# blacksnail789521/IMM-TSF

Measured on AMD Instinct MI355X. Metric: forecast windows/sec (train fwd+bwd) on ragged 64-entity batch, higher is better.
Workload: dtype bf16

## Files before the change

imm-tsf_amd/csrc/capi.hip:

```cpp
#include "../../include/immtsf.h"
#include "attn.hpp"
#include "gemm.hpp"
#include "rowops.hpp"
#include "tail.hpp"
#include "block_util.hpp"
#include <atomic>

namespace {
inline DropCfg mk_drop(float p, uint64_t seed) {
    DropCfg d;
    d.seed = seed;
    d.p = p > 0.f ? p : 0.f;
    d.inv_keep = d.p > 0.f ? 1.f / (1.f - d.p) : 1.f;
    d.seed_dev = nullptr;
    return d;
}
}

namespace { std::atomic<int> g_side_enabled{0}; }

extern "C" {

int immtsf_side_stream_enabled(void) { return g_side_enabled; }
int immtsf_set_side_stream(int32_t on) { g_side_enabled.store(on ? 1 : 0); return 0; }

int immtsf_gemm(int32_t layout, int32_t precision, const float* A, int32_t lda, const float* B, int32_t ldb, float* C,
                int32_t ldc, const float* bias, int32_t M, int32_t N, int32_t K, float alpha, int32_t accumulate,
                int32_t act, immtsf_stream_t stream) {
    if (!A || !B || !C || layout < 0 || layout > 2) return IMMTSF_EINVAL;
    GemmArgs g = gemm_args(M, N, K, lda, ldb, ldc);
    set_problem(g, 0, A, B, C, bias);
    g.alpha = alpha;
    g.accumulate = accumulate;
    g.act = act;
    return immtsf_launch_gemm(layout, precision, g, static_cast<hipStream_t>(stream));
}

int immtsf_linear_backward(int32_t precision, const float* x, const float* W, const float* dy, int32_t M, int32_t N,
                           int32_t K, float* dx, const float* relu_x, float* dW, float* db, int32_t grads_prezeroed,
                           immtsf_stream_t stream) {
    if (!dy || M <= 0 || N <= 0 || K <= 0 || (db && !dW) || (dx && !W) || (dW && !x)) return IMMTSF_EINVAL;
    hipStream_t s = static_cast<hipStream_t>(stream);
    if (linear_small_ok(M, N, K) && (!dW || grads_prezeroed)) return launch_linear_small_bwd(x, W, dy, M, N, K, dx, relu_x, dW, db, s);
    if (dx) {
        GemmArgs g = gemm_args(M, K, N, N, K, K);
        set_problem(g, 0, dy, W, dx, nullptr);
        g.relu_ref = relu_x;
        g.ld_ref = K;
        if (int rc = immtsf_launch_gemm(GEMM_NN, precision, g, s)) return rc;
    }
    if (dW) {
        GemmArgs g = gemm_args(N, K, M, N, K, K);
        set_problem(g, 0, dy, x, dW, nullptr, db);
        g.c_prezeroed = grads_prezeroed ? 1 : 0;
        if (int rc = immtsf_launch_gemm(GEMM_TN, precision, g, s)) return rc;
    }
// ... 78 lines not shown
    return launch_bf16_to_f32(src, dst, n, static_cast<hipStream_t>(stream));
}

int immtsf_gemm_batched(int32_t layout, int32_t precision, const float* A, int32_t lda, int64_t sA_o, int64_t sA_i,
                        const float* B, int32_t ldb, int64_t sB_o, int64_t sB_i, float* C, int32_t ldc, int64_t sC_o,
                        int64_t sC_i, int32_t n_outer, int32_t n_inner, int32_t M, int32_t N, int32_t K, float alpha,
                        immtsf_stream_t stream) {
    if (!A || !B || !C || layout < 0 || layout > 2 || n_outer <= 0 || n_inner <= 0) return IMMTSF_EINVAL;
    GemmArgs g = gemm_args(M, N, K, lda, ldb, ldc);
    set_problem(g, 0, A, B, C, nullptr);
    g.alpha = alpha;
    g.nbatch = n_outer * n_inner;
    g.batch_inner = n_inner;
    g.sA_o = sA_o; g.sA_i = sA_i; g.sB_o = sB_o; g.sB_i = sB_i; g.sC_o = sC_o; g.sC_i = sC_i;
    if (g.nbatch == 1) { g.nbatch = 1; }
    return immtsf_launch_gemm(layout, precision, g, static_cast<hipStream_t>(stream));
}

int immtsf_softmax_rows_forward(float* sc, float* A, int32_t B, int32_t H, int32_t L, int32_t S, const uint8_t* live,
                                float p_drop, uint64_t seed, uint64_t site, int32_t causal, const uint64_t* seed_step_dev,
                                immtsf_stream_t stream) {
    if (!sc || !A) return IMMTSF_EINVAL;
    DropCfg d = mk_drop(p_drop, seed);
    d.seed_dev = seed_step_dev;
    return launch_softmax_rows_fwd(sc, A, B, H, L, S, live, d, site, causal, static_cast<hipStream_t>(stream));
}

int immtsf_softmax_rows_backward(float* dA, const float* P, int32_t B, int32_t H, int32_t L, int32_t S, float p_drop,
                                 uint64_t seed, uint64_t site, const uint64_t* seed_step_dev, immtsf_stream_t stream) {
    if (!dA || !P) return IMMTSF_EINVAL;
    DropCfg d = mk_drop(p_drop, seed);
    d.seed_dev = seed_step_dev;
    return launch_softmax_rows_bwd(dA, P, B, H, L, S, d, site, static_cast<hipStream_t>(stream));
}

int immtsf_attention_short_forward(const float* qkv, int32_t B, int32_t L, int32_t H, int32_t E, float scale, int32_t causal,
                                   float p_drop, uint64_t seed, uint64_t site, const uint64_t* seed_step_dev, float* out,
                                   immtsf_stream_t stream) {
    if (!qkv || !out || B < 0 || L <= 0 || H <= 0 || E <= 0) return IMMTSF_EINVAL;
    DropCfg d = mk_drop(p_drop, seed);
    d.seed_dev = seed_step_dev;
    return launch_attn_short_fwd(qkv, B, L, H, E, scale, causal, d, site, out, static_cast<hipStream_t>(stream));
}

int immtsf_attention_short_backward(const float* qkv, const float* dout, int32_t B, int32_t L, int32_t H, int32_t E, float scale,
                                    int32_t causal, float p_drop, uint64_t seed, uint64_t site, const uint64_t* seed_step_dev,
                                    float* dqkv, immtsf_stream_t stream) {
    if (!qkv || !dout || !dqkv || B < 0 || L <= 0 || H <= 0 || E <= 0) return IMMTSF_EINVAL;
    DropCfg d = mk_drop(p_drop, seed);
    d.seed_dev = seed_step_dev;
    return launch_attn_short_bwd(qkv, dout, B, L, H, E, scale, causal, d, site, dqkv, static_cast<hipStream_t>(stream));
}

int immtsf_layernorm_forward(const float* x, int32_t rows, int32_t d, const float* gamma, const float* beta, float eps,
                             float* xhat, float* rstd, float* z, float p_drop, uint64_t seed, uint64_t site,
                             immtsf_stream_t stream) {
    if (!x || !gamma || !beta || !z || d <= 0) return IMMTSF_EINVAL;
    return launch_layernorm_fwd(x, rows, d, gamma, beta, eps, xhat, rstd, z, mk_drop(p_drop, seed), site,
                                static_cast<hipStream_t>(stream));
}

int immtsf_layernorm_backward(float* dz_dy, int32_t rows, int32_t d, const float* gamma, const float* xhat,
                              const float* rstd, float* dx, float* dgamma, float* dbeta, float* scratch, float p_drop,
                              uint64_t seed, uint64_t site, immtsf_stream_t stream) {
    if (!dz_dy || !gamma || !xhat || !rstd || !dx || d <= 0) return IMMTSF_EINVAL;
    hipStream_t s = static_cast<hipStream_t>(stream);
    CHECK(launch_layernorm_bwd(dz_dy, rows, d, gamma, xhat, rstd, dx, mk_drop(p_drop, seed), site, s));
    if (dgamma && dbeta) {
        if (!scratch) return IMMTSF_EINVAL;
        return launch_colsum2(dz_dy, xhat, rows, d, d, dgamma, dbeta, scratch, s);
    }
    if (dgamma) {
        if (!scratch) return IMMTSF_EINVAL;
        CHECK(launch_colsum(dz_dy, xhat, rows, nullptr, d, d, dgamma, 0, scratch, s));
    }
    if (dbeta) {
        if (!scratch) return IMMTSF_EINVAL;
        CHECK(launch_colsum(dz_dy, nullptr, rows, nullptr, d, d, dbeta, 0, scratch, s));
    }
    return IMMTSF_OK;
}

int immtsf_dropout_mask(uint64_t seed, uint64_t site, uint64_t n, float p_drop, uint8_t* out, immtsf_stream_t stream) {
    if (!out) return IMMTSF_EINVAL;
    return launch_dropout_mask(seed, site, (size_t)n, p_drop, out, static_cast<hipStream_t>(stream));
}

int immtsf_masked_mse_sums(const float* truth, const float* pred, const float* mask, int32_t rows, int32_t C,
                           float* err_sum, float* cnt, float* scratch, immtsf_stream_t stream) {
    if (!truth || !pred || !mask || !err_sum || !cnt || !scratch || rows < 0 || C <= 0) return IMMTSF_EINVAL;
    return launch_mse_sums(truth, pred, mask, rows, C, err_sum, cnt, scratch, static_cast<hipStream_t>(stream));
}

int immtsf_masked_mse(const float* truth, const float* pred, const float* mask, int32_t rows, int32_t C, const float* cnt_global,
                      float* err_sum, float* cnt, float* loss, float* dpred, float grad_scale, immtsf_stream_t stream) {
    if (!truth || !pred || !mask || !loss || rows < 0 || C <= 0) return IMMTSF_EINVAL;
    if ((int64_t)rows * C > IMMTSF_MSE_SMALL_MAX || C > 4096) return IMMTSF_EUNSUPPORTED;
    return launch_mse_small(truth, pred, mask, rows, C, cnt_global, err_sum, cnt, loss, dpred, grad_scale,
                            static_cast<hipStream_t>(stream));
}

int immtsf_masked_mse_counted(const float* truth, const float* pred, const float* mask, int32_t rows, int32_t C, const float* cnt_global,
                              float* scratch, float* loss, float* dpred, float grad_scale, immtsf_stream_t stream) {
    if (!truth || !pred || !mask || !cnt_global || !scratch || !loss || rows < 0 || C <= 0) return IMMTSF_EINVAL;
    if (C > 64) return IMMTSF_EUNSUPPORTED;
    return launch_mse_counted(truth, pred, mask, rows, C, cnt_global, scratch + 1, reinterpret_cast<unsigned int*>(scratch), loss, dpred,
// ... 117 lines not shown
```

imm-tsf_amd/csrc/rowops.hip:

```cpp
#include "rowops.hpp"

namespace {

constexpr int kSlabs = 32;

__global__ __launch_bounds__(256) void note_mask_kernel(const float* __restrict__ V, int rows, int d_m,
                                                         unsigned char* __restrict__ mask, int* nan_flag, int vec) {
    const int lane = threadIdx.x & 63, row = blockIdx.x * 4 + (threadIdx.x >> 6);
    if (row >= rows) return;
    const float* p = V + (size_t)row * d_m;
    float s = 0.f;
    bool bad = false;
    if (vec) {
        const float4* p4 = reinterpret_cast<const float4*>(p);
        for (int i = lane; i < d_m / 4; i += 64) {
            const float4 v = p4[i];
            s += fabsf(v.x) + fabsf(v.y) + fabsf(v.z) + fabsf(v.w);
            bad |= (v.x != v.x) | (v.y != v.y) | (v.z != v.z) | (v.w != v.w);
        }
    } else {
        for (int i = lane; i < d_m; i += 64) {
            const float v = p[i];
            s += fabsf(v);
            bad |= (v != v);
// ... 1484 lines not shown
        hipLaunchKernelGGL(layernorm_bwd_kernel, dim3(cdiv(rows, 4)), dim3(256), 0, s, dz_dy, rows, d, gamma, xhat, rstd, dx, drop,
                           site);
    IMMTSF_LAUNCH_CHECK();
    return IMMTSF_OK;
}

bool ln_sums_compact_ok(int rows, int d) {
    return (d & 3) == 0 && d <= 256 * LN_DV && rows >= 512 && (size_t)3 * 3 * d * sizeof(float) <= 64 * 1024;
}
int launch_layernorm_bwd_sums(float* dz_dy, int rows, int d, const float* gamma, const float* xhat, const float* rstd, float* dx,
                              DropCfg drop, uint64_t site, float* out_gw, float* out_gb, float* out_q, float* scratch,
                              const unsigned char* row_flag, int flag_div, void* dxh, hipStream_t s, const void* xhat_h) {
    if (rows <= 0) return IMMTSF_OK;
    constexpr bool on = true;
    const uintptr_t al = reinterpret_cast<uintptr_t>(dz_dy) | reinterpret_cast<uintptr_t>(dx) | reinterpret_cast<uintptr_t>(xhat) |
                         reinterpret_cast<uintptr_t>(gamma) | reinterpret_cast<uintptr_t>(scratch);
    if (!on || (d & 3) || d > 256 * LN_DV || (al & 15) || ((reinterpret_cast<uintptr_t>(dxh) | reinterpret_cast<uintptr_t>(xhat_h)) & 7) ||
        rows < 512)
        return IMMTSF_EUNSUPPORTED;
    if ((!xhat && !xhat_h) || (!dx && !dxh)) return IMMTSF_EINVAL;
    int nsl = (rows + 3) / 4;
    nsl = nsl > kLnSlabsMax ? kLnSlabsMax : nsl;
    const size_t lds = (size_t)3 * (out_q ? 3 : 2) * d * sizeof(float);
    if (out_q) {
        if (lds > 64 * 1024) return IMMTSF_EUNSUPPORTED;
        if (xhat_h)
            hipLaunchKernelGGL((layernorm_bwd_sums_kernel<3, true>), dim3(nsl), dim3(256), lds, s, dz_dy, rows, d, gamma, xhat_h, rstd, dx, drop, site,
                               scratch, row_flag, flag_div > 0 ? flag_div : 1, static_cast<bf16_t*>(dxh));
        else
            hipLaunchKernelGGL((layernorm_bwd_sums_kernel<3, false>), dim3(nsl), dim3(256), lds, s, dz_dy, rows, d, gamma, xhat, rstd, dx, drop, site,
                               scratch, row_flag, flag_div > 0 ? flag_div : 1, static_cast<bf16_t*>(dxh));
        IMMTSF_LAUNCH_CHECK();
        hipLaunchKernelGGL((colsum_vec_final_kernel<3>), dim3(cdiv(d, 32), 3), dim3(256), 0, s, scratch, d, nsl, out_gw, out_gb, out_q, 0);
    } else {
        if (lds > 64 * 1024 || row_flag || dxh || xhat_h || !dx) return IMMTSF_EUNSUPPORTED;
        hipLaunchKernelGGL((layernorm_bwd_sums_kernel<2, false>), dim3(nsl), dim3(256), lds, s, dz_dy, rows, d, gamma, xhat, rstd, dx, drop, site, scratch,
                           nullptr, 1, nullptr);
        IMMTSF_LAUNCH_CHECK();
        hipLaunchKernelGGL((colsum_vec_final_kernel<2>), dim3(cdiv(d, 32), 2), dim3(256), 0, s, scratch, d, nsl, out_gw, out_gb, nullptr, 0);
    }
    IMMTSF_LAUNCH_CHECK();
    return IMMTSF_OK;
}

int launch_instance_norm(const float* x, int B, int L, int C, float* xn, float* means, float* stdev, hipStream_t s) {
    if (B <= 0 || L <= 0 || C <= 0) return IMMTSF_OK;
    const size_t lds = ((size_t)L * C + 2 * (size_t)C) * sizeof(float);
    if (lds > 64 * 1024) return IMMTSF_EUNSUPPORTED;
    hipLaunchKernelGGL(instance_norm_kernel, dim3(B), dim3(256), lds, s, x, B, L, C, xn, means, stdev);
    IMMTSF_LAUNCH_CHECK();
    return IMMTSF_OK;
}

bool ln_lr_ok(int rows, int d, int PW) {
    return (d & 3) == 0 && d <= 1024 && d >= 256 && PW >= 1 && PW <= 64 && rows >= 512 && (size_t)(PW + 3) * d * sizeof(float) <= 150 * 1024;
}
int launch_layernorm_bwd_lr(const float* G, int ldg, int PW, const float* Wb, int rows, int d, const float* gamma, const float* xhat,
                            const void* xhat_h, const float* rstd, float* dx, void* dxh, DropCfg drop, uint64_t site, float* out_gw, float* out_gb,
                            float* out_q, float* scratch, const unsigned char* row_flag, int flag_div, hipStream_t s, const void* keep, int keep_T) {
    if (!ln_lr_ok(rows, d, PW)) return IMMTSF_EUNSUPPORTED;
    if (keep && (keep_T <= 0 || keep_T > 32)) return IMMTSF_EINVAL;
    if (!G || !Wb || (!xhat && !xhat_h) || (!dx && !dxh) || !out_gw || !out_gb || !out_q || !scratch) return IMMTSF_EINVAL;
    const uintptr_t al = reinterpret_cast<uintptr_t>(Wb) | reinterpret_cast<uintptr_t>(dx) | reinterpret_cast<uintptr_t>(gamma) |
                         reinterpret_cast<uintptr_t>(scratch) | reinterpret_cast<uintptr_t>(xhat);
    if ((al & 15) || ((reinterpret_cast<uintptr_t>(dxh) | reinterpret_cast<uintptr_t>(xhat_h)) & 7)) return IMMTSF_EUNSUPPORTED;
    const void* xa = xhat_h ? xhat_h : static_cast<const void*>(xhat);
    const size_t lds = (size_t)(PW + 3) * d * sizeof(float);
    const bool many = rows >= 8192;
    const int per_wg = 8 * (many ? (d <= 768 ? 4 : 2) : 1);
    int nsl = cdiv(rows, per_wg);
    nsl = nsl > 256 ? 256 : nsl;
    const int fd = flag_div > 0 ? flag_div : 1;
#define LNLR(RR, DVV, XHH)                                                                                                                       \
    do {                                                                                                                                         \
        static const hipError_t attr = hipFuncSetAttribute(reinterpret_cast<const void*>(layernorm_bwd_lr_kernel<RR, DVV, XHH>),                 \
                                                           hipFuncAttributeMaxDynamicSharedMemorySize, 150 * 1024);                              \
        if (attr != hipSuccess) return (int)attr;                                                                                                \
        hipLaunchKernelGGL((layernorm_bwd_lr_kernel<RR, DVV, XHH>), dim3(nsl), dim3(512), lds, s, G, ldg, PW, Wb, rows, d, gamma, xa, rstd, dx,   \
                           static_cast<bf16_t*>(dxh), drop, site, scratch, row_flag, fd, static_cast<const unsigned long long*>(keep), keep_T); \
    } while (0)
#define LNLR2(RR, DVV) do { if (xhat_h) LNLR(RR, DVV, true); else LNLR(RR, DVV, false); } while (0)
    if (d <= 768) { if (many) LNLR2(4, 3); else LNLR2(1, 3); }
    else { if (many) LNLR2(2, 4); else LNLR2(1, 4); }
#undef LNLR2
#undef LNLR
    IMMTSF_LAUNCH_CHECK();
    hipLaunchKernelGGL((colsum_vec_final_kernel<3>), dim3(cdiv(d, 32), 3), dim3(256), 0, s, scratch, d, nsl, out_gw, out_gb, out_q, 0);
    IMMTSF_LAUNCH_CHECK();
    return IMMTSF_OK;
}

int launch_matvec(const float* W, int ldw, const float* x, const float* b, int rows, int cols, float* y, float* ys,
                  float scale, hipStream_t s, float* y_nobias) {
    hipLaunchKernelGGL(matvec_kernel, dim3(cdiv(rows, 4)), dim3(256), 0, s, W, ldw, x, b, rows, cols, y, ys, scale, y_nobias);
    IMMTSF_LAUNCH_CHECK();
    return IMMTSF_OK;
}

int launch_matvec_t(const float* W, int ldw, const float* x, int rows, int cols, float* y, int accumulate,
                    hipStream_t s) {
    const int slabs = (accumulate && rows >= 256) ? 16 : 1;
    hipLaunchKernelGGL(matvec_t_kernel, dim3(cdiv(cols, 64), slabs), dim3(1024), 0, s, W, ldw, x, rows, cols, y, accumulate);
    IMMTSF_LAUNCH_CHECK();
    return IMMTSF_OK;
}

int launch_outer(const float* a, const float* b, int rows, int cols, float* out, int ld, hipStream_t s) {
    const long n = (long)rows * cols;
    hipLaunchKernelGGL(outer_kernel, dim3((unsigned)((n + 255) / 256)), dim3(256), 0, s, a, b, rows, cols, out, ld);
    IMMTSF_LAUNCH_CHECK();
    return IMMTSF_OK;
}

int launch_query_bwd(const float* dqs_part, int B, int d, float scale, const float* Wq, int ldw, const float* Q, float* dWq, int ldg,
                     float* dbq, float* dQ, hipStream_t s) {
    if (d <= 0) return IMMTSF_OK;
    hipLaunchKernelGGL(query_bwd_kernel, dim3(cdiv(d, QB_ROWS)), dim3(256), 0, s, dqs_part, B, d, scale, Wq, ldw, Q,
                       dWq, ldg, dbq, dQ);
    IMMTSF_LAUNCH_CHECK();
    return IMMTSF_OK;
}

int launch_query_t2v_bwd(const float* dqs_part, int B, int d, float scale, const float* Wq, int ldw, const float* Q, float* dWq, int ldg,
                         float* dbq, float* dQ, const float* tau_pad, const int* rowmap, const int* total, int max_rows, int d_tau,
                         const float* w, const float* b, const float* dfeat, int ld, float* dw0, float* db0, float* dw, float* db,
                         float* scratch, int nslabs, hipStream_t s, int accumulate) {
    if (d <= 0 || max_rows <= 0) return IMMTSF_EINVAL;
    if (nslabs < 1) nslabs = kSlabs;
    const int nq = cdiv(d, QB_ROWS), gx = cdiv(d_tau, 64);
    const QueryBwdJob q{dqs_part, B, d, scale, Wq, ldw, Q, dWq, ldg, dbq, dQ};
    const T2VBwdJob t{tau_pad, rowmap, total, d_tau, w, b, dfeat, ld, scratch, max_rows, gx, nslabs};
    hipLaunchKernelGGL(query_t2v_bwd_kernel, dim3(nq + gx * nslabs), dim3(256), 0, s, q, nq, t);
    IMMTSF_LAUNCH_CHECK();
    hipLaunchKernelGGL(time2vec_bwd_final_kernel, dim3(cdiv(d_tau, 4)), dim3(256), 0, s, scratch, d_tau, dw0, db0, dw, db, nslabs, accumulate);
    IMMTSF_LAUNCH_CHECK();
    return IMMTSF_OK;
// ... 90 lines not shown
```

imm-tsf_amd/csrc/rowops.hpp:

```cpp
#pragma once
#include "common.hpp"

int launch_note_mask(const float* V, int rows, int d_m, unsigned char* mask, int* nan_flag, hipStream_t s);
int launch_ragged_index(const unsigned char* mask, int B, int N, int* lengths, int* offsets, int* rowmap, int* seg,
                        unsigned char* mtxt, hipStream_t s, unsigned char* mtxt2 = nullptr);
int launch_mask_from_lengths(const int* lengths, int B, int N, unsigned char* mask, hipStream_t s);
int launch_gather_rows(const float* src, int ld_src, const int* rowmap, const int* total, int max_rows, int width,
                       float* dst, int ld_dst, hipStream_t s, void* dst_h = nullptr);
int launch_time2vec_fwd(const float* tau_pad, const int* rowmap, const int* total, int max_rows, int d_tau,
                        const float* w0, const float* b0, const float* w, const float* b, float* dst, int ld_dst,
                        hipStream_t s, void* dst_h = nullptr);
int launch_notes_stage(const float* src, int ld_src, const int* gmap, const int* total, int max_rows, int width, void* dst_h, int ld_dst,
                       const float* tau_pad, const int* rowmap, int d_tau, const float* w0, const float* b0, const float* w, const float* b,
                       float* t_dst, int t_ld, void* t_dst_h, const float* W, int ldw, const float* x, const float* bias, int rows, int cols,
                       float* y, float* ys, float scale, hipStream_t s,
                       const float* W2 = nullptr, int ldw2 = 0, const float* x2 = nullptr, const float* bias2 = nullptr, int rows2 = 0,
                       int cols2 = 0, float* y2 = nullptr,
                       const float* score_u = nullptr, float* score_out = nullptr);
int launch_query_t2v_bwd(const float* dqs_part, int B, int d, float scale, const float* Wq, int ldw, const float* Q, float* dWq, int ldg,
                         float* dbq, float* dQ, const float* tau_pad, const int* rowmap, const int* total, int max_rows, int d_tau,
                         const float* w, const float* b, const float* dfeat, int ld, float* dw0, float* db0, float* dw, float* db,
                         float* scratch, int nslabs, hipStream_t s, int accumulate = 0);
int launch_time2vec_bwd(const float* tau_pad, const int* rowmap, const int* total, int max_rows, int d_tau,
                        const float* w, const float* b, const float* dfeat, int ld, float* dw0, float* db0, float* dw,
                        float* db, float* scratch, int nslabs, hipStream_t s, int accumulate = 0);
int launch_colsum(const float* X, const float* Y, int M, const int* dyn, int N, int ld, float* out, int accumulate,
                  float* scratch, hipStream_t s, bool big_scratch = false);
bool colsum_small_pair_ok(int M, int N);
int launch_colsum_small_pair(const float* X, const float* Y, const float* Z, int M, int N, int ld, float* out_xy, float* out_x, float* out_z,
                             hipStream_t s, int outputs_zero = 0);
int launch_colsum2(const float* X, const float* Y, int M, int N, int ld, float* out_xy, float* out_x, float* scratch,
                   hipStream_t s, bool big_scratch = false);
inline size_t colsum_scratch_floats(size_t ncols, int k) { return (size_t)256 * k * ((ncols + 3) & ~(size_t)3) + 64 * 8; }
int launch_colsum3(const float* X, const float* Y, float* Z, int M, int N, int ld, float* out_xy, float* out_x, float* out_z,
                   float* scratch, const unsigned char* row_flag, int flag_div, void* Zh, hipStream_t s, bool big_scratch = false);
int launch_layernorm_fwd(const float* x, int rows, int d, const float* gamma, const float* beta, float eps, float* xhat,
                         float* rstd, float* z, DropCfg drop, uint64_t site, hipStream_t s, void* zh = nullptr,
                         const float* res = nullptr, DropCfg pre = DropCfg{0, 0.f, 1.f, nullptr}, uint64_t presite = 0,
                         void* xhat_h = nullptr);
int launch_layernorm_bwd(float* dz_dy, int rows, int d, const float* gamma, const float* xhat, const float* rstd,
                         float* dx, DropCfg drop, uint64_t site, hipStream_t s, float* dbranch = nullptr,
                         DropCfg pre = DropCfg{0, 0.f, 1.f, nullptr}, uint64_t presite = 0);
constexpr int kLnSlabsMax = 2048;
inline size_t ln_sums_scratch_floats(size_t d, int k) { return (size_t)kLnSlabsMax * k * ((d + 3) & ~(size_t)3) + 64 * 8; }
int launch_layernorm_bwd_sums(float* dz_dy, int rows, int d, const float* gamma, const float* xhat, const float* rstd, float* dx,
                              DropCfg drop, uint64_t site, float* out_gw, float* out_gb, float* out_q, float* scratch,
                              const unsigned char* row_flag, int flag_div, void* dxh, hipStream_t s, const void* xhat_h = nullptr);
int launch_instance_norm(const float* x, int B, int L, int C, float* xn, float* means, float* stdev, hipStream_t s);
bool ln_lr_ok(int rows, int d, int PW);
int launch_layernorm_bwd_lr(const float* G, int ldg, int PW, const float* Wb, int rows, int d, const float* gamma, const float* xhat,
                            const void* xhat_h, const float* rstd, float* dx, void* dxh, DropCfg drop, uint64_t site, float* out_gw, float* out_gb,
                            float* out_q, float* scratch, const unsigned char* row_flag, int flag_div, hipStream_t s, const void* keep = nullptr,
                            int keep_T = 0);
bool ln_sums_compact_ok(int rows, int d);
int launch_matvec(const float* W, int ldw, const float* x, const float* b, int rows, int cols, float* y, float* ys,
                  float scale, hipStream_t s, float* y_nobias = nullptr);
int launch_matvec_t(const float* W, int ldw, const float* x, int rows, int cols, float* y, int accumulate,
                    hipStream_t s);
int launch_outer(const float* a, const float* b, int rows, int cols, float* out, int ld, hipStream_t s);
int launch_axpy(const float* src, float alpha, float* dst, int n, int accumulate, hipStream_t s);
int launch_query_bwd(const float* dqs_part, int B, int d, float scale, const float* Wq, int ldw, const float* Q, float* dWq, int ldg,
                     float* dbq, float* dQ, hipStream_t s);
int launch_fill(float* dst, float v, size_t n, hipStream_t s);
int launch_dropout_mask(uint64_t seed, uint64_t site, size_t n, float p, unsigned char* out, hipStream_t s);
bool head_sums_supported(int M, int C);
int launch_head_sums(const float* dn, const float* xhat, const float* ddelta, const unsigned char* flag, int flag_div, int M, int C,
                     float* out_xy, float* out_x, float* slive, hipStream_t s);
int launch_head_outer(const float* Wres, int d, const float* slive, const float* bout, int C, float* dbout, float* dWres, hipStream_t s);
```

imm-tsf_amd/csrc/xrank.hip:

```cpp
#include "../../include/immtsf.h"
#include "gemm.hpp"
#include "rowops.hpp"
#include "tail.hpp"
#include "block_util.hpp"
#include "t2v_fold.hpp"
#include "eval.hpp"
#include <math.h>
#include <algorithm>
#include <vector>
#include <type_traits>

namespace {

constexpr int XR = 8;
constexpr int XJ_MAX = 20;
enum { XJ_NN = 0, XJ_NT = 1, XJ_OUTER = 2, XJ_COPY = 3 };
struct XJob {
    int form, nblk;
    const float* L; int lsr, lsn;
    int R;
    const float* W; int ldw, qsn;
    int K, N, M;
    float* out; int osr, osn;
    unsigned short* out16;
    float alpha;
    const float *lb, *wb;
    const float* radd;
    const float* xrow;
    int ng; long pgs, qgs;
};
struct XJobs { int first[XJ_MAX]; int n; int lds_floats; XJob j[XJ_MAX]; };

__device__ __forceinline__ unsigned short f2bf(float v) {
    return __builtin_bit_cast(unsigned short, static_cast<__bf16>(v));
}

constexpr int XJ_LK = 16 * 1024;

__device__ __forceinline__ bool xjob_stage_l(const XJob& J, float* Ls, int cap) {
    if (J.R * J.K > cap) return false;
    if (J.lsn == 1) {
        for (int i = threadIdx.x; i < J.R * J.K; i += 256) {
            const int r = i / J.K, k = i - r * J.K;
            Ls[i] = J.L[(size_t)r * J.lsr + k];
        }
    } else {
        for (int i = threadIdx.x; i < J.R * J.K; i += 256) {
            const int k = i / J.R, r = i - k * J.R;
            Ls[r * J.K + k] = J.L[(size_t)r * J.lsr + (size_t)k * J.lsn];
        }
    }
    __syncthreads();
    return true;
}

template <bool STAGED>
__device__ __forceinline__ void xjob_nn_acc(const XJob& J, int kg, int n, const float* Ls, float4 (&acc)[XR]) {
    constexpr int U = STAGED ? 8 : 6;
    const int R = J.R;
// ... 1411 lines not shown
    }
    {
        GemmArgs g = gemm_args(BT, x.PW, d, d, d, x.PW);
        set_problem2(g, 0, Em, mat(w.Wf, w.Wf16), mat(P), w.Wfb);
        CHECK(immtsf_launch_gemm(GEMM_NT, prec, g, s));
    }
    return IMMTSF_OK;
}

static int xrank_compose_z(const immtsf_fusion_cfg* cfg, const float* proj_w, const float* proj_b, const XPWs& w, hipStream_t s) {
    const XRDims x = xr_dims(cfg);
    const int d = x.d, prec = cfg->precision;
    const bool hf = xr_hf(cfg);
    Mat Wpo;
    CHECK(weight_mat(hf, proj_w, (size_t)d * d, w.Wpo16, s, &Wpo));
    {
        GemmArgs g = gemm_args(x.PW, d, d, d, d, d);
        set_problem2(g, 0, mat(w.Wf, w.Wf16), Wpo, mat(w.Wc, w.Wc16), nullptr);
        CHECK(immtsf_launch_gemm(GEMM_NN, prec, g, s));
    }
    {
        VecJobList l;
        l.add(VJ_MV, w.Wf, d, proj_b, w.Wfb, w.bc, x.PW, d);
        CHECK(launch_vecjobs(l, s));
    }
    return IMMTSF_OK;
}

int immtsf_mmf_xrank_fold_z(const immtsf_fusion_cfg* cfg, const immtsf_xadd_params* p, const float* proj_w, const float* proj_b, float* bHO,
                            void* workspace, size_t workspace_bytes, immtsf_stream_t stream) {
    if (!proj_w || !proj_b) return IMMTSF_EINVAL;
    CHECK(immtsf_mmf_xrank_fold(cfg, p, bHO, workspace, workspace_bytes, stream));
    return xrank_compose_z(cfg, proj_w, proj_b, carve_xp(cfg, workspace), static_cast<hipStream_t>(stream));
}

int immtsf_mmf_xrank_p_forward_z(const immtsf_fusion_cfg* cfg, const immtsf_xadd_params* p, const float* proj_w, const float* proj_b,
                                 const float* Z, float* P, float* bHO, void* workspace, size_t workspace_bytes, int32_t folded,
                                 immtsf_stream_t stream) {
    if (!xr_supported(cfg) || !p || !proj_w || !proj_b || !Z || !P || !bHO || !workspace) return IMMTSF_EINVAL;
    XPWs w = carve_xp(cfg, workspace);
    if (workspace_bytes < w.bytes) return IMMTSF_EWORKSPACE;
    if (!folded) CHECK(immtsf_mmf_xrank_fold_z(cfg, p, proj_w, proj_b, bHO, workspace, workspace_bytes, stream));
    hipStream_t s = static_cast<hipStream_t>(stream);
    const XRDims x = xr_dims(cfg);
    const int d = x.d, BT = x.B * x.T, prec = cfg->precision;
    const bool hf = xr_hf(cfg);
    Mat Zm = cmat(Z);
    if (hf && cfg->in_h) {
        Zm.h = const_cast<void*>(cfg->in_h);
    } else if (hf) {
        CHECK(launch_f32_to_bf16(Z, w.E16, (size_t)BT * d, s));
        Zm.h = w.E16;
    }
    {
        GemmArgs g = gemm_args(BT, x.PW, d, d, d, x.PW);
        set_problem2(g, 0, Zm, mat(w.Wc, w.Wc16), mat(P), w.bc);
        CHECK(immtsf_launch_gemm(GEMM_NT, prec, g, s));
    }
    return IMMTSF_OK;
}

int immtsf_mmf_xrank_p_backward_data_z(const immtsf_fusion_cfg* cfg, const immtsf_xadd_params* p, const float* proj_w, const float* proj_b,
                                       const float* Z, const float* dP, float* dZ, void* workspace, size_t workspace_bytes, void* scratch,
                                       size_t scratch_bytes, immtsf_stream_t stream) {
    if (!xr_supported(cfg) || !p || !proj_w || !proj_b || !Z || !dP || !dZ || !workspace || !scratch) return IMMTSF_EINVAL;
    XPWs w = carve_xp(cfg, workspace);
    XPScratch sc = carve_xp_scratch(cfg, scratch);
    if (workspace_bytes < w.bytes || scratch_bytes < sc.bytes) return IMMTSF_EWORKSPACE;
    hipStream_t s = static_cast<hipStream_t>(stream);
    const XRDims x = xr_dims(cfg);
    const int d = x.d, BT = x.B * x.T, prec = cfg->precision;
    const bool hf = xr_hf(cfg);
    Mat Wpo;
    CHECK(weight_mat(hf, proj_w, (size_t)d * d, w.Wpo16, s, &Wpo));
    Mat dPm = cmat(dP), Zm = cmat(Z, hf ? (cfg->aux_h ? cfg->aux_h : static_cast<const void*>(w.E16)) : nullptr);
    const bool seed_only = cfg->bwd_phase != 0 && !(cfg->bwd_phase & IMMTSF_BWD_PHASE_A);
    if (hf && !cfg->aux_h && !seed_only) CHECK(launch_f32_to_bf16(Z, w.E16, (size_t)BT * d, s));
    if (hf && cfg->in_h) {
        dPm.h = const_cast<void*>(cfg->in_h);
    } else if (hf) {
        if (!seed_only) CHECK(launch_f32_to_bf16(dP, sc.dP16, (size_t)BT * x.PW, s));
        dPm.h = sc.dP16;
    }
    const bool do_data = cfg->bwd_phase == 0 || (cfg->bwd_phase & IMMTSF_BWD_PHASE_A), do_seed = cfg->bwd_phase == 0 || (cfg->bwd_phase & IMMTSF_BWD_WGRAD_A);
    if (do_data && !(cfg->form & IMMTSF_FORM_LOWRANK_OUT)) {
        if (rank_expand_ok(BT, d, x.PW, w.Wc, d, dZ, hf ? cfg->out_h : nullptr)) {
            CHECK(launch_rank_expand(dP, x.PW, w.Wc, d, dZ, hf ? cfg->out_h : nullptr, BT, d, x.PW, s));
        } else {
            GemmArgs g = gemm_args(BT, d, x.PW, x.PW, d, d);
            set_problem2(g, 0, dPm, mat(w.Wc, w.Wc16), mat(dZ, hf ? cfg->out_h : nullptr), nullptr);
            CHECK(immtsf_launch_gemm(GEMM_NN, prec, g, s));
        }
    }
    if (do_seed) {
        GemmArgs g = gemm_args(x.PW, d, BT, x.PW, d, d);
        set_problem2(g, 0, dPm, Zm, mat(sc.dWc), nullptr, sc.dbc);
        g.c_prezeroed = 0;
        g.ws = sc.sk; g.ws_bytes = sc.skb;
        CHECK(immtsf_launch_gemm(GEMM_TN, prec, g, s));
        if (hf) CHECK(launch_f32_to_bf16(sc.dWc, sc.dWc16, (size_t)x.PW * d, s));
    }
    return IMMTSF_OK;
}

int immtsf_mmf_xrank_lowrank_basis(const immtsf_fusion_cfg* cfg, void* workspace, size_t workspace_bytes, const float** basis, int32_t* rank) {
    if (!xr_supported(cfg) || !workspace || !basis || !rank) return IMMTSF_EINVAL;
    XPWs w = carve_xp(cfg, workspace);
// ... 251 lines not shown
```

imm-tsf_amd/immtsf/_lib.py:

```python
from __future__ import annotations

import ctypes as C
import os

_HERE = os.path.dirname(os.path.abspath(__file__))
LIB_PATH = os.path.join(_HERE, "libimmtsf_hip.so")

ABI_VERSION = 7
FORM_NO_PROJ = 16
FORM_HALF_OUT = 32
FORM_LOWRANK_OUT = 64
BWD_PHASE_A, BWD_PHASE_B, BWD_PHASE_C = 1, 2, 4
BWD_WGRAD_A, BWD_WGRAD_B, BWD_WGRAD_C = 16, 32, 64


class ImmtsfError(RuntimeError):
    pass


_ERR = {-1: "IMMTSF_EINVAL (bad dimension / null pointer)", -2: "IMMTSF_EWORKSPACE (workspace too small)",
        -3: "IMMTSF_EUNSUPPORTED (shape outside kernel limits)"}

c_f32p = C.c_void_p
c_u8p = C.c_void_p
# ... 358 lines not shown
                                                  C.c_float, C.c_uint64, C.c_uint64, C.c_void_p, c_f32p, c_stream]),
    "immtsf_layernorm_forward": (C.c_int, [c_f32p, C.c_int32, C.c_int32, c_f32p, c_f32p, C.c_float, c_f32p, c_f32p,
                                           c_f32p, C.c_float, C.c_uint64, C.c_uint64, c_stream]),
    "immtsf_layernorm_backward": (C.c_int, [c_f32p, C.c_int32, C.c_int32, c_f32p, c_f32p, c_f32p, c_f32p, c_f32p, c_f32p,
                                            c_f32p, C.c_float, C.c_uint64, C.c_uint64, c_stream]),
    "immtsf_dropout_mask": (C.c_int, [C.c_uint64, C.c_uint64, C.c_uint64, C.c_float, c_u8p, c_stream]),
    "immtsf_set_side_stream": (C.c_int, [C.c_int32]),
    "immtsf_side_stream_enabled": (C.c_int, []),
    "immtsf_flag_set": (C.c_int, [C.c_void_p, c_stream]),
    "immtsf_flag_wait": (C.c_int, [C.c_void_p, C.c_void_p, C.c_int32, c_stream]),
    "immtsf_flags_clear": (C.c_int, [C.c_void_p, C.c_int32, c_stream]),
    "immtsf_flags_clear_set": (C.c_int, [C.c_void_p, C.c_int32, C.c_void_p, c_stream]),
    "immtsf_flag_bump": (C.c_int, [C.c_void_p, c_stream]),
    "immtsf_flag_wait_ge": (C.c_int, [C.c_void_p, C.c_int32, C.c_void_p, C.c_int32, c_stream]),
    "immtsf_flag_trace": (C.c_int, [C.c_int32]),
    "immtsf_flag_trace_read": (C.c_int, [C.c_void_p, C.c_int32]),
    "immtsf_timing_enable": (C.c_int, [C.c_int32]),
    "immtsf_debug_gemm_config": (C.c_int, [C.c_int32, C.c_int32]),
    "immtsf_timing_collect": (C.c_int, [C.c_int32, C.c_void_p, C.c_void_p, C.c_void_p]),
    "immtsf_gemm_bf16_group_tn": (C.c_int, [C.c_int32, C.c_void_p, C.c_void_p, C.c_void_p, C.c_void_p, C.c_void_p, C.c_void_p, C.c_void_p,
                                            C.c_void_p, C.c_void_p, c_stream]),
    "immtsf_embed_forward": (C.c_int, [C.c_int32, c_f32p] + [C.c_int32] * 7 + [c_f32p, c_f32p, c_f32p, C.c_float, C.c_uint64, C.c_uint64,
                                       C.c_void_p, c_stream]),
    "immtsf_embed_backward": (C.c_int, [C.c_int32, c_f32p] + [C.c_int32] * 7 + [c_f32p, c_f32p, c_f32p, C.c_int32, c_f32p, C.c_float,
                                        C.c_uint64, C.c_uint64, C.c_void_p, c_stream]),
    "immtsf_gemm_bf16": (C.c_int, [C.c_int32, C.c_void_p, C.c_int32, C.c_void_p, C.c_int32, c_f32p, C.c_int32, C.c_void_p,
                                   C.c_int32, c_f32p, c_f32p, C.c_int32, C.c_int32, C.c_int32, C.c_float, C.c_int32, C.c_int32,
                                   c_i32p, C.c_int32, c_i32p, c_stream]),
    "immtsf_debug_gemm2_config": (C.c_int, [C.c_int32, C.c_int32, C.c_int32]),
    "immtsf_gemm3_bf16": (C.c_int, [C.c_int32, C.c_void_p, C.c_int32, C.c_void_p, C.c_int32, c_f32p, C.c_int32, C.c_void_p,
                                    C.c_int32, c_f32p, c_f32p, c_i32p, C.c_int32, C.c_int32, C.c_int32, C.c_int32, C.c_float,
                                    C.c_int32, c_i32p, c_stream]),
    "immtsf_debug_gemm3_config": (C.c_int, [C.c_int32, C.c_int32]),
    "immtsf_gemm3_tn_workspace_bytes": (C.c_size_t, [C.c_int32, C.c_int32, C.c_int32]),
    "immtsf_gemm3_tn_bf16": (C.c_int, [C.c_void_p, C.c_int32, C.c_void_p, C.c_int32, c_f32p, C.c_int32, c_f32p, C.c_int32, C.c_int32,
                                       C.c_int32, C.c_float, C.c_int32, c_i32p, C.c_void_p, C.c_size_t, c_stream]),
    "immtsf_adam_step_dev": (C.c_int, [c_f32p, c_f32p, c_f32p, c_f32p, C.c_uint64, C.c_float, C.c_float, C.c_float,
                                       C.c_float, C.c_float, C.c_void_p, C.c_float, c_f32p, C.c_void_p, c_stream]),
    "immtsf_adam_step_dev_zero": (C.c_int, [c_f32p, c_f32p, c_f32p, c_f32p, C.c_uint64, C.c_float, C.c_float, C.c_float,
                                       C.c_float, C.c_float, C.c_void_p, C.c_float, c_f32p, C.c_void_p, c_stream]),
    "immtsf_adam_step_guarded": (C.c_int, [c_f32p, c_f32p, c_f32p, c_f32p, C.c_uint64, C.c_float, C.c_float, C.c_float,
                                           C.c_float, C.c_float, C.c_void_p, C.c_float, c_f32p, C.c_void_p, C.c_void_p, C.c_int32, c_stream]),
    "immtsf_adam_sqnorm": (C.c_int, [c_f32p, C.c_uint64, c_f32p, C.c_void_p, C.c_void_p, c_stream]),
    "immtsf_adam_apply": (C.c_int, [c_f32p, c_f32p, c_f32p, c_f32p, C.c_uint64, C.c_float, C.c_float, C.c_float, C.c_float, C.c_float,
                                    C.c_int32, C.c_void_p, C.c_float, c_f32p, C.c_void_p, c_stream]),
    "immtsf_adam_step": (C.c_int, [c_f32p, c_f32p, c_f32p, c_f32p, C.c_uint64, C.c_float, C.c_float, C.c_float,
                                   C.c_float, C.c_float, C.c_int32, C.c_float, c_f32p, c_stream]),
    "immtsf_adam_prepare": (C.c_int, [c_f32p, C.c_void_p, C.c_uint64, c_f32p, C.c_void_p, C.c_void_p, C.c_void_p, C.c_void_p, C.c_void_p,
                                      c_f32p, C.c_void_p, c_stream]),
    "immtsf_flag_wait_ge_multi": (C.c_int, [C.c_int32, C.c_void_p, C.c_int32, C.c_void_p, C.c_int32, C.c_void_p, C.c_int32, c_stream]),
    "immtsf_adam_range": (C.c_int, [c_f32p, c_f32p, C.c_void_p, c_f32p, c_f32p, C.c_uint64, C.c_uint64, C.c_uint64, C.c_float, C.c_float,
                                    C.c_float, C.c_float, C.c_float, C.c_void_p, C.c_float, c_f32p, C.c_int32, C.c_void_p, c_stream]),
    "immtsf_guard_pack": (C.c_int, [C.c_void_p, C.c_void_p, C.c_int32, c_stream]),
}

def abi_structs():
    return [FusionCfg, T2VParams, RecAvgParams, XAddParams, GRParams, TTCNParams, GCNParams, DecoderParams, Time2VecParams,
            EncoderLayerCfg, EncoderLayerParams, FFNBlockCfg, FFNBlockParams, Store, NoteIndex, LowRankGrad, LatentODEDims, NeuralFlowDims]


_lib = None


def load():
    global _lib
    if _lib is not None:
        return _lib
    global LIB_PATH
    LIB_PATH = os.environ.get("IMMTSF_LIB", LIB_PATH)
    if not os.path.exists(LIB_PATH):
        raise ImmtsfError(
            f"{LIB_PATH} not found: build it with `python -c 'import __graft_entry__ as g; g.build()'` "
            f"or `make -C imm-tsf_amd/csrc`.  There is no CPU fallback.")
    lib = C.CDLL(LIB_PATH)
    for name, (res, args) in _PROTOS.items():
        try:
            fn = getattr(lib, name)
        except AttributeError as e:
            raise ImmtsfError(f"{LIB_PATH} does not export {name}; rebuild it") from e
        fn.restype = res
        fn.argtypes = args
    if lib.immtsf_abi_version() != ABI_VERSION:
        raise ImmtsfError("libimmtsf_hip.so ABI version mismatch; rebuild it")
    structs = abi_structs()
    sizes = (C.c_int32 * len(structs))()
    if lib.immtsf_abi_sizes(sizes, len(structs)) != len(structs) or any(int(sizes[i]) != C.sizeof(t) for i, t in enumerate(structs)):
        raise ImmtsfError("libimmtsf_hip.so struct layout differs from this binding (immtsf_abi_sizes); rebuild it")
    _lib = lib
    return lib


def exported_names():
    return sorted(_PROTOS)


def check(rc: int, what: str):
    if rc == 0:
        return
    if rc < 0:
        raise ImmtsfError(f"{what}: {_ERR.get(rc, rc)}")
    raise ImmtsfError(f"{what}: hipError_t {rc}")


def ptr(t):
    return None if t is None else C.c_void_p(t.data_ptr())

# ... 5 lines not shown
```

include/immtsf.h:

```cpp
#ifndef IMMTSF_H
#define IMMTSF_H

#include <stddef.h>
#include <stdint.h>

#ifdef __cplusplus
extern "C" {
#endif

#define IMMTSF_ABI_VERSION 7
#define IMMTSF_T2V_FOLD_MIN_ROWS 8192
#define IMMTSF_FORM_NO_PROJ 16
#define IMMTSF_FORM_HALF_OUT 32
#define IMMTSF_FORM_LOWRANK_OUT 64

#define IMMTSF_OK 0
#define IMMTSF_EINVAL (-1)
#define IMMTSF_EWORKSPACE (-2)
#define IMMTSF_EUNSUPPORTED (-3)

typedef void* immtsf_stream_t;

int immtsf_abi_version(void);
int immtsf_instance_norm(const float* x, int32_t B, int32_t L, int32_t C, float* xn, float* means, float* stdev, immtsf_stream_t stream);
// ... 474 lines not shown
int immtsf_collate_patches(const immtsf_store* s, const int32_t* window_ids, int32_t B, int32_t npatch, float patch_size,
                           float patch_stride, float history, int32_t Lp, float time_max, float* obs_tp, float* obs_data,
                           float* obs_mask, immtsf_stream_t stream);
int immtsf_collate_union(const immtsf_store* s, const int32_t* window_ids, int32_t B, const float* axis, int32_t T, int32_t n_obs,
                         float time_max, float* obs_tp, float* obs_data, float* obs_mask, float* pred_tp, float* pred_data,
                         float* pred_mask, immtsf_stream_t stream);
int immtsf_collate_notes(const immtsf_store* s, const int32_t* window_ids, int32_t B, int32_t Nmax, float* tau, float* notes,
                         int32_t* lengths, int32_t* offsets, int32_t* rowmap, immtsf_stream_t stream);

int immtsf_collate_batch(const immtsf_store* s, const int32_t* window_ids, int32_t B, int32_t Lmax, int32_t Lpmax, int32_t Nmax,
                         float time_max, float* obs_tp, float* obs_data, float* obs_mask, float* pred_tp, float* pred_data,
                         float* pred_mask, float* tau, float* notes, int32_t* lengths, int32_t* offsets, int32_t* rowmap,
                         immtsf_stream_t stream);
int immtsf_collate_patch_max(const immtsf_store* s, int32_t W, int32_t npatch, float patch_size, float patch_stride, float history,
                             int32_t* out, immtsf_stream_t stream);

int immtsf_gemm(int32_t layout, int32_t precision, const float* A, int32_t lda, const float* B, int32_t ldb, float* C,
                int32_t ldc, const float* bias, int32_t M, int32_t N, int32_t K, float alpha, int32_t accumulate,
                int32_t act, immtsf_stream_t stream);
int immtsf_linear_backward(int32_t precision, const float* x, const float* W, const float* dy, int32_t M, int32_t N,
                           int32_t K, float* dx, const float* relu_x, float* dW, float* db, int32_t grads_prezeroed,
                           immtsf_stream_t stream);
int immtsf_time2vec_forward(const float* t, int32_t rows, int32_t d, const float* w0, const float* b0, const float* w,
                            const float* b, float* out, immtsf_stream_t stream);
int immtsf_time2vec_backward(const float* t, int32_t rows, int32_t d, const float* w, const float* b, const float* dout,
                             float* dw0, float* db0, float* dw, float* db, float* scratch, int32_t accumulate,
                             immtsf_stream_t stream);
int immtsf_bf16_twin_register(const float* base, void* twin, size_t count);
int immtsf_bf16_twin_unregister(const float* base);
int immtsf_bf16_twin_enable(int32_t on);
int immtsf_f32_to_bf16(const float* src, void* dst, size_t n, immtsf_stream_t stream);
int immtsf_bf16_to_f32(const void* src, float* dst, size_t n, immtsf_stream_t stream);
int immtsf_linear_bf16_forward(int32_t nl, const float* x, void* x16, const float* const* W, void* const* w16, const float* const* b,
                               float* const* y, int32_t M, int32_t N, int32_t K, int32_t act, immtsf_stream_t stream);
int immtsf_linear_bf16_backward(int32_t nl, const void* x16, const float* const* W, void* const* w16, const float* const* dy, void* dy16,
                                float* dx, float* const* dW, float* const* db, int32_t M, int32_t N, int32_t K,
                                int32_t grads_prezeroed, immtsf_stream_t stream);
int immtsf_gemm_batched(int32_t layout, int32_t precision, const float* A, int32_t lda, int64_t sA_o, int64_t sA_i,
                        const float* B, int32_t ldb, int64_t sB_o, int64_t sB_i, float* C, int32_t ldc, int64_t sC_o,
                        int64_t sC_i, int32_t n_outer, int32_t n_inner, int32_t M, int32_t N, int32_t K, float alpha,
                        immtsf_stream_t stream);
int immtsf_softmax_rows_forward(float* sc, float* A, int32_t B, int32_t H, int32_t L, int32_t S, const uint8_t* live,
                                float p_drop, uint64_t seed, uint64_t site, int32_t causal, const uint64_t* seed_step_dev,
                                immtsf_stream_t stream);
int immtsf_softmax_rows_backward(float* dA, const float* P, int32_t B, int32_t H, int32_t L, int32_t S, float p_drop,
                                 uint64_t seed, uint64_t site, const uint64_t* seed_step_dev, immtsf_stream_t stream);
#define IMMTSF_ATTN_SHORT_MAX 8
int immtsf_attention_short_forward(const float* qkv, int32_t B, int32_t L, int32_t H, int32_t E, float scale, int32_t causal,
                                   float p_drop, uint64_t seed, uint64_t site, const uint64_t* seed_step_dev, float* out,
                                   immtsf_stream_t stream);
int immtsf_attention_short_backward(const float* qkv, const float* dout, int32_t B, int32_t L, int32_t H, int32_t E, float scale,
                                    int32_t causal, float p_drop, uint64_t seed, uint64_t site, const uint64_t* seed_step_dev,
                                    float* dqkv, immtsf_stream_t stream);
int immtsf_layernorm_forward(const float* x, int32_t rows, int32_t d, const float* gamma, const float* beta, float eps,
                             float* xhat, float* rstd, float* z, float p_drop, uint64_t seed, uint64_t site,
                             immtsf_stream_t stream);
int immtsf_layernorm_backward(float* dz_dy, int32_t rows, int32_t d, const float* gamma, const float* xhat,
                              const float* rstd, float* dx, float* dgamma, float* dbeta, float* scratch,
                              float p_drop, uint64_t seed, uint64_t site, immtsf_stream_t stream);
int immtsf_dropout_mask(uint64_t seed, uint64_t site, uint64_t n, float p_drop, uint8_t* out, immtsf_stream_t stream);
#define IMMTSF_SITE_T2V_ATTN 1
#define IMMTSF_SITE_T2V_OUT 2
#define IMMTSF_SITE_REC_OUT 3
#define IMMTSF_SITE_XADD_ATTN 4
#define IMMTSF_SITE_XADD_OUT 5
#define IMMTSF_SITE_GR_OUT 6
#define IMMTSF_SITE_LAYER_BASE 16

int immtsf_adam_step(float* param, const float* grad, float* exp_avg, float* exp_avg_sq, uint64_t n, float lr,
                     float beta1, float beta2, float eps, float weight_decay, int32_t step, float max_norm,
                     float* norm_scratch, immtsf_stream_t stream);
int immtsf_adam_step_dev(float* param, const float* grad, float* exp_avg, float* exp_avg_sq, uint64_t n, float lr,
                         float beta1, float beta2, float eps, float weight_decay, int64_t* step_dev, float max_norm,
                         float* norm_scratch, uint64_t* dropout_step_dev, immtsf_stream_t stream);

int immtsf_adam_step_dev_zero(float* param, float* grad, float* exp_avg, float* exp_avg_sq, uint64_t n, float lr, float beta1,
                              float beta2, float eps, float weight_decay, int64_t* step_dev, float max_norm, float* norm_scratch,
                              uint64_t* dropout_step_dev, immtsf_stream_t stream);

int immtsf_adam_step_guarded(float* param, float* grad, float* exp_avg, float* exp_avg_sq, uint64_t n, float lr, float beta1,
                             float beta2, float eps, float weight_decay, int64_t* step_dev, float max_norm, float* norm_scratch,
                             uint64_t* dropout_step_dev, const int32_t* skip_flag, int32_t zero_grad, immtsf_stream_t stream);

int immtsf_adam_sqnorm(const float* grad, uint64_t n, float* norm_scratch, int64_t* step_dev, uint64_t* dropout_step_dev,
                       immtsf_stream_t stream);
int immtsf_adam_apply(float* param, const float* grad, float* exp_avg, float* exp_avg_sq, uint64_t n, float lr, float beta1,
                      float beta2, float eps, float weight_decay, int32_t step, const int64_t* step_dev, float max_norm,
                      const float* norm_scratch, void* twin, immtsf_stream_t stream);

int immtsf_adam_prepare(const float* grad, const void* grad_h, uint64_t n, float* norm_scratch, int64_t* step_dev,
                        uint64_t* dropout_step_dev, int32_t* pending, const int32_t* err, const void* guard_h, const float* guard_f,
                        int32_t* skip_out, immtsf_stream_t stream);
int immtsf_adam_range(float* param, float* grad, const void* grad_h, float* exp_avg, float* exp_avg_sq, uint64_t n, uint64_t lo,
                      uint64_t hi, float lr, float beta1, float beta2, float eps, float weight_decay, const int64_t* step_dev,
                      float max_norm, const float* norm_scratch, int32_t zero_grad, const int32_t* skip, immtsf_stream_t stream);
int immtsf_guard_pack(const int32_t* err, void* slot, int32_t is_bf16, immtsf_stream_t stream);

typedef struct immtsf_encoder_layer_cfg {
    int32_t Bs, S, D, H, F;
    int32_t precision, training;
    float p_attn, p_drop, eps;
    uint64_t seed;
    const uint64_t* seed_step_dev;
    uint64_t site_base;
    int32_t grads_prezeroed;
} immtsf_encoder_layer_cfg;
// ... 132 lines not shown
```

Baseline: 151,600.

## Add MFMA skinny projection kernel and multi-row layernorm backward for mid-size batches

Adds a dedicated bf16 MFMA kernel for the small-width output projection (PW ≤ 64) used when row counts fall between 512 and 8192. It splits the K dimension across four waves and reduces the partial sums through LDS, replacing the generic GEMM path. It also lets the low-rank layernorm backward process two rows per lane group for mid-size batches instead of one, and exposes new C API entry points. The aim is to cut launch and tile inefficiency of the general GEMM on skinny shapes, at the cost of extra code paths and lower occupancy per workgroup.

```diff
diff --git a/imm-tsf_amd/csrc/capi.hip b/imm-tsf_amd/csrc/capi.hip
--- a/imm-tsf_amd/csrc/capi.hip
+++ b/imm-tsf_amd/csrc/capi.hip
@@ -2,6 +2,7 @@
 #include "attn.hpp"
 #include "gemm.hpp"
 #include "rowops.hpp"
+#include "seam_small.hpp"
 #include "tail.hpp"
 #include "block_util.hpp"
 #include <atomic>
@@ -186,6 +187,22 @@
     return launch_attn_short_bwd(qkv, dout, B, L, H, E, scale, causal, d, site, dqkv, static_cast<hipStream_t>(stream));
 }
 
+int immtsf_seam_route(int32_t rows, int32_t d, int32_t PW) { return seam_p_fwd_shape_ok(rows, d, PW) ? 1 : 0; }
+
+int immtsf_seam_p_bf16(const void* A, const void* W, const float* bias, float* P, int32_t rows, int32_t d, int32_t PW, immtsf_stream_t stream) {
+    return launch_seam_p_fwd(A, W, bias, P, rows, d, PW, static_cast<hipStream_t>(stream));
+}
+
+int immtsf_layernorm_backward_lowrank(const float* G, int32_t ldg, int32_t PW, const float* basis, int32_t rows, int32_t d, const float* gamma,
+                                      const float* xhat, const void* xhat_h, const float* rstd, float* dx, void* dxh, float p_drop,
+                                      const void* keep, int32_t keep_T, const uint8_t* row_flag, int32_t flag_div, float* dgamma, float* dbeta,
+                                      float* dxsum, float* scratch, size_t scratch_bytes, int32_t form, immtsf_stream_t stream) {
+    if (scratch_bytes < (size_t)256 * 3 * d * sizeof(float) || (form != 0 && form != 1)) return IMMTSF_EINVAL;
+    if (p_drop > 0.f && !keep) return IMMTSF_EINVAL;
+    return launch_layernorm_bwd_lr(G, ldg, PW, basis, rows, d, gamma, xhat, xhat_h, rstd, dx, dxh, mk_drop(p_drop, 0), 0, dgamma, dbeta, dxsum,
+                                   scratch, row_flag, flag_div, static_cast<hipStream_t>(stream), keep, keep_T, form);
+}
+
 int immtsf_layernorm_forward(const float* x, int32_t rows, int32_t d, const float* gamma, const float* beta, float eps,
                              float* xhat, float* rstd, float* z, float p_drop, uint64_t seed, uint64_t site,
                              immtsf_stream_t stream) {
diff --git a/imm-tsf_amd/csrc/rowops.hip b/imm-tsf_amd/csrc/rowops.hip
--- a/imm-tsf_amd/csrc/rowops.hip
+++ b/imm-tsf_amd/csrc/rowops.hip
@@ -1560,12 +1560,16 @@
     return IMMTSF_OK;
 }
 
+#ifndef LNLR_SMALL_R
+#define LNLR_SMALL_R 2
+#endif
 bool ln_lr_ok(int rows, int d, int PW) {
     return (d & 3) == 0 && d <= 1024 && d >= 256 && PW >= 1 && PW <= 64 && rows >= 512 && (size_t)(PW + 3) * d * sizeof(float) <= 150 * 1024;
 }
 int launch_layernorm_bwd_lr(const float* G, int ldg, int PW, const float* Wb, int rows, int d, const float* gamma, const float* xhat,
                             const void* xhat_h, const float* rstd, float* dx, void* dxh, DropCfg drop, uint64_t site, float* out_gw, float* out_gb,
-                            float* out_q, float* scratch, const unsigned char* row_flag, int flag_div, hipStream_t s, const void* keep, int keep_T) {
+                            float* out_q, float* scratch, const unsigned char* row_flag, int flag_div, hipStream_t s, const void* keep, int keep_T,
+                            int form) {
     if (!ln_lr_ok(rows, d, PW)) return IMMTSF_EUNSUPPORTED;
     if (keep && (keep_T <= 0 || keep_T > 32)) return IMMTSF_EINVAL;
     if (!G || !Wb || (!xhat && !xhat_h) || (!dx && !dxh) || !out_gw || !out_gb || !out_q || !scratch) return IMMTSF_EINVAL;
@@ -1575,7 +1579,8 @@
     const void* xa = xhat_h ? xhat_h : static_cast<const void*>(xhat);
     const size_t lds = (size_t)(PW + 3) * d * sizeof(float);
     const bool many = rows >= 8192;
-    const int per_wg = 8 * (many ? (d <= 768 ? 4 : 2) : 1);
+    const int R = form == 1 ? 1 : many ? (d <= 768 ? 4 : 2) : (d <= 768 ? LNLR_SMALL_R : 2);
+    const int per_wg = 8 * R;
     int nsl = cdiv(rows, per_wg);
     nsl = nsl > 256 ? 256 : nsl;
     const int fd = flag_div > 0 ? flag_div : 1;
@@ -1588,8 +1593,8 @@
                            static_cast<bf16_t*>(dxh), drop, site, scratch, row_flag, fd, static_cast<const unsigned long long*>(keep), keep_T); \
     } while (0)
 #define LNLR2(RR, DVV) do { if (xhat_h) LNLR(RR, DVV, true); else LNLR(RR, DVV, false); } while (0)
-    if (d <= 768) { if (many) LNLR2(4, 3); else LNLR2(1, 3); }
-    else { if (many) LNLR2(2, 4); else LNLR2(1, 4); }
+    if (d <= 768) { if (R == 4) LNLR2(4, 3); else if (R == 2) LNLR2(2, 3); else LNLR2(1, 3); }
+    else { if (R == 2) LNLR2(2, 4); else LNLR2(1, 4); }
 #undef LNLR2
 #undef LNLR
     IMMTSF_LAUNCH_CHECK();
diff --git a/imm-tsf_amd/csrc/rowops.hpp b/imm-tsf_amd/csrc/rowops.hpp
--- a/imm-tsf_amd/csrc/rowops.hpp
+++ b/imm-tsf_amd/csrc/rowops.hpp
@@ -51,7 +51,7 @@
 int launch_layernorm_bwd_lr(const float* G, int ldg, int PW, const float* Wb, int rows, int d, const float* gamma, const float* xhat,
                             const void* xhat_h, const float* rstd, float* dx, void* dxh, DropCfg drop, uint64_t site, float* out_gw, float* out_gb,
                             float* out_q, float* scratch, const unsigned char* row_flag, int flag_div, hipStream_t s, const void* keep = nullptr,
-                            int keep_T = 0);
+                            int keep_T = 0, int form = 0);
 bool ln_sums_compact_ok(int rows, int d);
 int launch_matvec(const float* W, int ldw, const float* x, const float* b, int rows, int cols, float* y, float* ys,
                   float scale, hipStream_t s, float* y_nobias = nullptr);
diff --git a/imm-tsf_amd/csrc/seam_small.hip b/imm-tsf_amd/csrc/seam_small.hip
--- /dev/null
+++ b/imm-tsf_amd/csrc/seam_small.hip
@@ -0,0 +1,82 @@
+#include "seam_small.hpp"
+
+namespace {
+
+template <int NT>
+__global__ __launch_bounds__(256) void seam_p_fwd_kernel(const bf16_t* __restrict__ A, const bf16_t* __restrict__ W, const float* __restrict__ bias,
+                                                          float* __restrict__ out, int rows, int d, int PW) {
+    __shared__ f32x4 red[3][NT][64];
+    const int tid = threadIdx.x, lane = tid & 63, wave = tid >> 6, fr = lane & 15, fq = lane >> 4;
+    const int row = blockIdx.x * 16 + fr;
+    const bool rok = row < rows;
+    const bf16_t* ap = A + (size_t)(rok ? row : 0) * d + fq * 8;
+    const bf16_t* wp[NT];
+    bool wok[NT];
+#pragma unroll
+    for (int j = 0; j < NT; ++j) {
+        wok[j] = j * 16 + fr < PW;
+        wp[j] = W + (size_t)(wok[j] ? j * 16 + fr : 0) * d + fq * 8;
+    }
+    f32x4 acc[NT];
+#pragma unroll
+    for (int j = 0; j < NT; ++j) acc[j] = f32x4{0.f, 0.f, 0.f, 0.f};
+    bf16x8 zero;
+#pragma unroll
+    for (int e = 0; e < 8; ++e) zero[e] = (bf16_t)0.0f;
+    const int nk = d >> 5;
+#pragma unroll 4
+    for (int ks = wave; ks < nk; ks += 4) {
+        const bf16x8 a = rok ? *reinterpret_cast<const bf16x8*>(ap + ks * 32) : zero;
+#pragma unroll
+        for (int j = 0; j < NT; ++j) {
+            const bf16x8 b = wok[j] ? *reinterpret_cast<const bf16x8*>(wp[j] + ks * 32) : zero;
+            acc[j] = __builtin_amdgcn_mfma_f32_16x16x32_bf16(a, b, acc[j], 0, 0, 0);
+        }
+    }
+    if (wave > 0) {
+#pragma unroll
+        for (int j = 0; j < NT; ++j) red[wave - 1][j][lane] = acc[j];
+    }
+    __syncthreads();
+    if (wave > 0) return;
+#pragma unroll
+    for (int j = 0; j < NT; ++j) {
+#pragma unroll
+        for (int w = 0; w < 3; ++w) acc[j] += red[w][j][lane];
+        const int n = j * 16 + fr;
+        if (n >= PW) continue;
+        const float b = bias ? bias[n] : 0.f;
+#pragma unroll
+        for (int r = 0; r < 4; ++r) {
+            const int orow = blockIdx.x * 16 + fq * 4 + r;
+            if (orow < rows) out[(size_t)orow * PW + n] = acc[j][r] + b;
+        }
+    }
+}
+
+constexpr int SEAM_MIN_ROWS = 512, SEAM_MAX_ROWS = 8192;
+
+}
+
+bool seam_p_fwd_shape_ok(int rows, int d, int PW) {
+    return rows >= SEAM_MIN_ROWS && rows < SEAM_MAX_ROWS && PW >= 1 && PW <= 64 && d >= 32 && d <= 1024 && (d & 31) == 0;
+}
+bool seam_p_fwd_ok(int rows, int d, int PW, const void* A, const void* W, const void* out) {
+    const uintptr_t al = reinterpret_cast<uintptr_t>(A) | reinterpret_cast<uintptr_t>(W);
+    return seam_p_fwd_shape_ok(rows, d, PW) && (al & 15) == 0 && A && W && out;
+}
+
+int launch_seam_p_fwd(const void* A, const void* W, const float* bias, float* out, int rows, int d, int PW, hipStream_t s) {
+    if (!seam_p_fwd_ok(rows, d, PW, A, W, out)) return IMMTSF_EUNSUPPORTED;
+    const bf16_t* a = static_cast<const bf16_t*>(A);
+    const bf16_t* w = static_cast<const bf16_t*>(W);
+    const dim3 grid((rows + 15) / 16);
+    switch ((PW + 15) / 16) {
+        case 1: hipLaunchKernelGGL((seam_p_fwd_kernel<1>), grid, dim3(256), 0, s, a, w, bias, out, rows, d, PW); break;
+        case 2: hipLaunchKernelGGL((seam_p_fwd_kernel<2>), grid, dim3(256), 0, s, a, w, bias, out, rows, d, PW); break;
+        case 3: hipLaunchKernelGGL((seam_p_fwd_kernel<3>), grid, dim3(256), 0, s, a, w, bias, out, rows, d, PW); break;
+        default: hipLaunchKernelGGL((seam_p_fwd_kernel<4>), grid, dim3(256), 0, s, a, w, bias, out, rows, d, PW); break;
+    }
+    IMMTSF_LAUNCH_CHECK();
+    return IMMTSF_OK;
+}
diff --git a/imm-tsf_amd/csrc/seam_small.hpp b/imm-tsf_amd/csrc/seam_small.hpp
--- /dev/null
+++ b/imm-tsf_amd/csrc/seam_small.hpp
@@ -0,0 +1,6 @@
+#pragma once
+#include "common.hpp"
+
+bool seam_p_fwd_shape_ok(int rows, int d, int PW);
+bool seam_p_fwd_ok(int rows, int d, int PW, const void* A, const void* W, const void* out);
+int launch_seam_p_fwd(const void* A, const void* W, const float* bias, float* out, int rows, int d, int PW, hipStream_t s);
diff --git a/imm-tsf_amd/csrc/xrank.hip b/imm-tsf_amd/csrc/xrank.hip
--- a/imm-tsf_amd/csrc/xrank.hip
+++ b/imm-tsf_amd/csrc/xrank.hip
@@ -5,6 +5,7 @@
 #include "block_util.hpp"
 #include "t2v_fold.hpp"
 #include "eval.hpp"
+#include "seam_small.hpp"
 #include <math.h>
 #include <algorithm>
 #include <vector>
@@ -1522,7 +1523,9 @@
         CHECK(launch_f32_to_bf16(Z, w.E16, (size_t)BT * d, s));
         Zm.h = w.E16;
     }
-    {
+    if (hf && seam_p_fwd_ok(BT, d, x.PW, Zm.h, w.Wc16, P)) {
+        CHECK(launch_seam_p_fwd(Zm.h, w.Wc16, w.bc, P, BT, d, x.PW, s));
+    } else {
         GemmArgs g = gemm_args(BT, x.PW, d, d, d, x.PW);
         set_problem2(g, 0, Zm, mat(w.Wc, w.Wc16), mat(P), w.bc);
         CHECK(immtsf_launch_gemm(GEMM_NT, prec, g, s));
diff --git a/imm-tsf_amd/immtsf/_lib.py b/imm-tsf_amd/immtsf/_lib.py
--- a/imm-tsf_amd/immtsf/_lib.py
+++ b/imm-tsf_amd/immtsf/_lib.py
@@ -434,6 +434,11 @@
     "immtsf_adam_range": (C.c_int, [c_f32p, c_f32p, C.c_void_p, c_f32p, c_f32p, C.c_uint64, C.c_uint64, C.c_uint64, C.c_float, C.c_float,
                                     C.c_float, C.c_float, C.c_float, C.c_void_p, C.c_float, c_f32p, C.c_int32, C.c_void_p, c_stream]),
     "immtsf_guard_pack": (C.c_int, [C.c_void_p, C.c_void_p, C.c_int32, c_stream]),
+    "immtsf_seam_route": (C.c_int, [C.c_int32] * 3),
+    "immtsf_seam_p_bf16": (C.c_int, [C.c_void_p, C.c_void_p, c_f32p, c_f32p, C.c_int32, C.c_int32, C.c_int32, c_stream]),
+    "immtsf_layernorm_backward_lowrank": (C.c_int, [c_f32p, C.c_int32, C.c_int32, c_f32p, C.c_int32, C.c_int32, c_f32p, c_f32p, C.c_void_p, c_f32p,
+                                                    c_f32p, C.c_void_p, C.c_float, C.c_void_p, C.c_int32, C.c_void_p, C.c_int32, c_f32p, c_f32p,
+                                                    c_f32p, c_f32p, C.c_size_t, C.c_int32, c_stream]),
 }
 
 def abi_structs():
diff --git a/include/immtsf.h b/include/immtsf.h
--- a/include/immtsf.h
+++ b/include/immtsf.h
@@ -550,6 +550,12 @@
 int immtsf_attention_short_backward(const float* qkv, const float* dout, int32_t B, int32_t L, int32_t H, int32_t E, float scale,
                                     int32_t causal, float p_drop, uint64_t seed, uint64_t site, const uint64_t* seed_step_dev,
                                     float* dqkv, immtsf_stream_t stream);
+int immtsf_seam_route(int32_t rows, int32_t d, int32_t PW);
+int immtsf_seam_p_bf16(const void* A, const void* W, const float* bias, float* P, int32_t rows, int32_t d, int32_t PW, immtsf_stream_t stream);
+int immtsf_layernorm_backward_lowrank(const float* G, int32_t ldg, int32_t PW, const float* basis, int32_t rows, int32_t d, const float* gamma,
+                                      const float* xhat, const void* xhat_h, const float* rstd, float* dx, void* dxh, float p_drop,
+                                      const void* keep, int32_t keep_T, const uint8_t* row_flag, int32_t flag_div, float* dgamma, float* dbeta,
+                                      float* dxsum, float* scratch, size_t scratch_bytes, int32_t form, immtsf_stream_t stream);
 int immtsf_layernorm_forward(const float* x, int32_t rows, int32_t d, const float* gamma, const float* beta, float eps,
                              float* xhat, float* rstd, float* z, float p_drop, uint64_t seed, uint64_t site,
                              immtsf_stream_t stream);
```

Result: faster. 155,800 (median of 6 runs) (+2.8%).
